# ReaganCardoza/Physics-Based-Ray-Tracing

Measured on AMD Instinct MI355X. Metric: Msamples/s on cbox.xml 512x512 x 256 spp (radiance, path max_depth 6), higher is better.
Workload: dtype f32

## Files before the change

### include/pbrt_hip.h

```cpp
#ifndef PBRT_HIP_H
#define PBRT_HIP_H

#include <stdint.h>

#ifdef __cplusplus
extern "C" {
#endif

#define PBRT_ABI_VERSION 5

#define PBRT_OK 0
#define PBRT_E_INVALID (-1)
#define PBRT_E_DEVICE (-2)
#define PBRT_E_NOMEM (-3)
#define PBRT_E_UNSUPPORTED (-4)

#define PBRT_PRIM_TRIANGLE 0u
#define PBRT_PRIM_SPHERE 1u
#define PBRT_PRIM_PARALLELOGRAM 2u
#define PBRT_PRIM_CONE 3u
#define PBRT_PRIM_CYLINDER 4u

typedef struct pbrt_prim {
    float g[12];
// ... 4 lines not shown
} pbrt_prim;

#define PBRT_MAT_DIFFUSE 0u
#define PBRT_MAT_CONDUCTOR 1u
#define PBRT_MAT_DIELECTRIC 2u
#define PBRT_MAT_ULTRA 3u
#define PBRT_MAT_NONE 4u
#define PBRT_MAT_ROUGHCONDUCTOR 5u
#define PBRT_MAT_CONDUCTOR_FRESNEL 6u

typedef struct pbrt_material {
    uint32_t type;
    float p[7];
} pbrt_material;

#define PBRT_EMIT_AREA 0u
#define PBRT_EMIT_POINT 1u

typedef struct pbrt_emitter {
    uint32_t type;
    float radiance[3];
    float pos[3];
    uint32_t first;
    uint32_t count;
    float area;
    float pad[2];
} pbrt_emitter;

#define PBRT_ACCEL_AUTO 0u
#define PBRT_ACCEL_BRUTE 1u
#define PBRT_ACCEL_BVH 2u
#define PBRT_ACCEL_BVH_GLOBAL 3u

typedef struct pbrt_scene_desc {
    uint32_t n_prims;
    const pbrt_prim *prims;
    uint32_t n_materials;
    const pbrt_material *materials;
    uint32_t n_emitters;
    const pbrt_emitter *emitters;
    uint32_t n_light_prims;
    const uint32_t *light_prims;
    const float *light_cdf;
    uint32_t accel;
    const float *vertex_normals;
} pbrt_scene_desc;

typedef struct pbrt_camera {
    float to_world[12];
    float tan_half_fov_x;
    float near_clip;
    float far_clip;
    uint32_t film_w;
    uint32_t film_h;
} pbrt_camera;

#define PBRT_FILTER_BOX 0u
#define PBRT_FILTER_TENT 1u
#define PBRT_FILTER_GAUSSIAN 2u

typedef struct pbrt_film_desc {
    uint32_t crop_x, crop_y, crop_w, crop_h;
    uint32_t spp;
    uint32_t sample_offset;
    uint32_t max_depth;
    uint32_t rr_depth;
    uint32_t filter;
    uint32_t seed;
    uint32_t flags;
    uint32_t pass_paths;
} pbrt_film_desc;

#define PBRT_FILM_RAW_ACCUM 1u
#define PBRT_FILM_NO_REPACK 2u
#define PBRT_FILM_FUSE_PLAN_SET 0x80u
#define PBRT_FILM_FUSE_PLAN(mask) (PBRT_FILM_FUSE_PLAN_SET | (((mask) & 0xffu) << 8))
#define PBRT_FILM_WALK_SET 0x10000u
#define PBRT_FILM_WALK_FROM(d) (PBRT_FILM_WALK_SET | (((d) & 0xffu) << 17))
#define PBRT_FILM_REGEN 8u
#define PBRT_FILM_NO_HIT_POOL 0x10u
#define PBRT_FILM_NO_OCCLUDER_PRUNING 4u
#define PBRT_FILM_NO_TILE_CULL 0x20u
#define PBRT_FILM_NO_ORDERED_WALK 0x40u

#define PBRT_US_MAX_ANGLES 64

typedef struct pbrt_us_emitter {
    uint32_t number_of_elements;
    float pitch, element_width, element_height;
    float radius;
    float opening_angle;
    uint32_t number_of_rays_per_element;
    float speed_of_sound;
    float steering_angle_min, steering_angle_max;
} pbrt_us_emitter;

#define PBRT_US_PRIMARY_ELEMENT 0u
#define PBRT_US_PRIMARY_EMITTER 1u
#define PBRT_US_ARRAY_CONVEX 0x100u

typedef struct pbrt_us_params {
    uint32_t max_depth;
    float frequency;
    float sound_speed;
    float attenuation;
    float main_beam_angle;
    float cutoff_angle;
    float fs;
    uint32_t n_elements;
    float pitch;
    uint32_t n_angles;
    float angles_deg[PBRT_US_MAX_ANGLES];
    uint32_t time_samples;
    float sensor_to_world[12];
    float max_path_len;
    uint32_t quirks;
    uint32_t primary;
    pbrt_us_emitter emitter;
} pbrt_us_params;

#define PBRT_USQ_DIAG_SAMPLE 0x1u
#define PBRT_USQ_REF_REFLECT 0x2u
#define PBRT_USQ_UNIT_GGX_PDF 0x4u
#define PBRT_USQ_DOUBLE_LOCAL 0x8u
#define PBRT_USQ_MIXED_FRAMES 0x10u
#define PBRT_USQ_NEVER_ENTER 0x20u
#define PBRT_USQ_CLAMP_TIME 0x40u
#define PBRT_USQ_NO_TOF_ACCUM 0x80u
#define PBRT_USQ_NO_CARRIER 0x100u
#define PBRT_USQ_NO_FIRST_TABLES 0x200u
#define PBRT_USQ_NO_FUSED_BOUNCES 0x400u
#define PBRT_USQ_FROZEN_DRAWS 0x800u
#define PBRT_USQ_SIGNED_RR 0x1000u
#define PBRT_USQ_DRJIT_VARIANT (PBRT_USQ_CLAMP_TIME | PBRT_USQ_NO_TOF_ACCUM | PBRT_USQ_FROZEN_DRAWS | PBRT_USQ_SIGNED_RR)
#define PBRT_USQ_REFERENCE                                                                \
    (PBRT_USQ_DIAG_SAMPLE | PBRT_USQ_REF_REFLECT | PBRT_USQ_UNIT_GGX_PDF | PBRT_USQ_DOUBLE_LOCAL | \
     PBRT_USQ_MIXED_FRAMES | PBRT_USQ_NEVER_ENTER)

typedef struct pbrt_us_sensor {
    uint32_t num_elements;
    float element_width, element_height, pitch;
    float radius;
    float center_frequency, sound_speed, directivity;
    float to_world[12];
} pbrt_us_sensor;

typedef struct pbrt_us_receiver {
    uint32_t number_of_elements;
    float pitch;
    float sample_rate;
    uint32_t time_samples;
} pbrt_us_receiver;

typedef struct pbrt_stats {
    uint64_t samples;
    uint64_t segments;
    uint64_t shadow_rays;
    double kernel_ms;
    double bounce_ms;
    uint32_t bounce_launches;
    uint32_t passes;
    uint64_t model_bytes;
    uint64_t bounce_model_bytes;
    uint64_t live[16];
    uint32_t fuse_plan;
    uint32_t plan_source;
// ... 223 lines not shown
```

### physics-based-ray-tracing_amd/_capi.py

```python
from __future__ import annotations

import contextlib
import ctypes as C
import os
import sys

import numpy as np

_HERE = os.path.dirname(os.path.abspath(__file__))
LIB_PATH = os.environ.get("PBRT_HIP_LIB") or os.path.join(_HERE, "csrc", "libpbrt_hip.so")

PBRT_ABI_VERSION = 5

PRIM_TRIANGLE, PRIM_SPHERE, PRIM_PARALLELOGRAM, PRIM_CONE, PRIM_CYLINDER = 0, 1, 2, 3, 4
MAT_DIFFUSE, MAT_CONDUCTOR, MAT_DIELECTRIC, MAT_ULTRA, MAT_NONE = 0, 1, 2, 3, 4
MAT_ROUGHCONDUCTOR, MAT_CONDUCTOR_FRESNEL = 5, 6
EMIT_AREA, EMIT_POINT = 0, 1
ACCEL_AUTO, ACCEL_BRUTE, ACCEL_BVH, ACCEL_BVH_GLOBAL = 0, 1, 2, 3
FILTER_BOX, FILTER_TENT, FILTER_GAUSSIAN = 0, 1, 2
FILM_RAW_ACCUM = 1
FILM_NO_REPACK = 2
FILM_NO_OCCLUDER_PRUNING = 4
FILM_NO_TILE_CULL = 0x20
FILM_NO_ORDERED_WALK = 0x40
FILM_NO_HIT_POOL = 0x10
FILM_REGEN = 8
FILM_FUSE_PLAN_SET = 0x80


FILM_WALK_SET = 0x10000


def film_walk_from(depth: int) -> int:
    return FILM_WALK_SET | ((int(depth) & 0xFF) << 17)


def film_fuse_plan(mask: int) -> int:
    return FILM_FUSE_PLAN_SET | ((int(mask) & 0xFF) << 8)

US_MAX_ANGLES = 64

USQ_DIAG_SAMPLE = 0x1
USQ_REF_REFLECT = 0x2
USQ_UNIT_GGX_PDF = 0x4
USQ_DOUBLE_LOCAL = 0x8
USQ_MIXED_FRAMES = 0x10
USQ_NEVER_ENTER = 0x20
USQ_CLAMP_TIME = 0x40
USQ_NO_TOF_ACCUM = 0x80
USQ_NO_CARRIER = 0x100
USQ_NO_FIRST_TABLES = 0x200
USQ_NO_FUSED_BOUNCES = 0x400
USQ_FROZEN_DRAWS = 0x800
USQ_SIGNED_RR = 0x1000
USQ_DRJIT_VARIANT = USQ_CLAMP_TIME | USQ_NO_TOF_ACCUM | USQ_FROZEN_DRAWS | USQ_SIGNED_RR
USQ_REFERENCE = (USQ_DIAG_SAMPLE | USQ_REF_REFLECT | USQ_UNIT_GGX_PDF | USQ_DOUBLE_LOCAL
                 | USQ_MIXED_FRAMES | USQ_NEVER_ENTER)

PRIM_DTYPE = np.dtype([("g", np.float32, 12), ("type", np.uint32), ("material", np.uint32),
                       ("emitter", np.int32), ("shape", np.uint32)])
MATERIAL_DTYPE = np.dtype([("type", np.uint32), ("p", np.float32, 7)])
EMITTER_DTYPE = np.dtype([("type", np.uint32), ("radiance", np.float32, 3), ("pos", np.float32, 3),
                          ("first", np.uint32), ("count", np.uint32), ("area", np.float32),
                          ("pad", np.float32, 2)])
assert PRIM_DTYPE.itemsize == 64 and MATERIAL_DTYPE.itemsize == 32 and EMITTER_DTYPE.itemsize == 48


class Material(C.Structure):
    _fields_ = [("type", C.c_uint32), ("p", C.c_float * 7)]


class SceneDesc(C.Structure):
    _fields_ = [("n_prims", C.c_uint32), ("prims", C.c_void_p),
                ("n_materials", C.c_uint32), ("materials", C.c_void_p),
                ("n_emitters", C.c_uint32), ("emitters", C.c_void_p),
                ("n_light_prims", C.c_uint32), ("light_prims", C.c_void_p), ("light_cdf", C.c_void_p),
                ("accel", C.c_uint32), ("vertex_normals", C.c_void_p)]


class Camera(C.Structure):
    _fields_ = [("to_world", C.c_float * 12), ("tan_half_fov_x", C.c_float), ("near_clip", C.c_float),
                ("far_clip", C.c_float), ("film_w", C.c_uint32), ("film_h", C.c_uint32)]


class FilmDesc(C.Structure):
    _fields_ = [("crop_x", C.c_uint32), ("crop_y", C.c_uint32), ("crop_w", C.c_uint32), ("crop_h", C.c_uint32),
                ("spp", C.c_uint32), ("sample_offset", C.c_uint32), ("max_depth", C.c_uint32),
                ("rr_depth", C.c_uint32), ("filter", C.c_uint32), ("seed", C.c_uint32), ("flags", C.c_uint32),
                ("pass_paths", C.c_uint32)]


class UsEmitter(C.Structure):
    _fields_ = [("number_of_elements", C.c_uint32), ("pitch", C.c_float), ("element_width", C.c_float),
                ("element_height", C.c_float), ("radius", C.c_float), ("opening_angle", C.c_float),
                ("number_of_rays_per_element", C.c_uint32), ("speed_of_sound", C.c_float),
                ("steering_angle_min", C.c_float), ("steering_angle_max", C.c_float)]


class UsParams(C.Structure):
    _fields_ = [("max_depth", C.c_uint32), ("frequency", C.c_float), ("sound_speed", C.c_float),
                ("attenuation", C.c_float), ("main_beam_angle", C.c_float), ("cutoff_angle", C.c_float),
                ("fs", C.c_float), ("n_elements", C.c_uint32), ("pitch", C.c_float), ("n_angles", C.c_uint32),
                ("angles_deg", C.c_float * US_MAX_ANGLES), ("time_samples", C.c_uint32),
                ("sensor_to_world", C.c_float * 12), ("max_path_len", C.c_float), ("quirks", C.c_uint32),
                ("primary", C.c_uint32), ("emitter", UsEmitter)]


# ... 460 lines not shown
```

### physics-based-ray-tracing_amd/csrc/diag_driver.h

```cpp
#pragma once

#ifndef PBRT_DEFAULT_WALK_FROM
#define PBRT_DEFAULT_WALK_FROM 0xffu
#endif

static RadKern diag_walk_kernel(const pbrt_scene *s, bool first, uint32_t nb) {
    return with_flags(
        [](auto F, auto B, auto N) -> RadKern { return &k_walk<F(), B() ? ACCEL_K_BRUTE_BIG : ACCEL_K_BRUTE, N() ? 2 : 1>; }, first,
        s->accel_kernel != ACCEL_K_BRUTE, nb == 2);
}
static RadKern diag_bvh_kernel(const pbrt_scene *s, bool first) {
    return with_flags([](auto F, auto L) -> RadKern { return &k_bounce<F(), L() ? ACCEL_K_BVH_LDS : ACCEL_K_BVH_GLOBAL>; }, first,
                      s->accel_kernel == ACCEL_K_BVH_LDS);
}
static UsKern diag_us_bvh_kernel(const pbrt_scene *s, bool first, bool convex) {
    return with_flags([](auto F, auto L, auto X) -> UsKern {
        return &k_us_bounce<F(), L() ? ACCEL_K_BVH_LDS : ACCEL_K_BVH_GLOBAL, false, US_Q_RUNTIME, -1, X()>; },
                      first, s->accel_kernel == ACCEL_K_BVH_LDS, convex);
}
static int diag_lds_attr(pbrt_scene *s, bool us) {
    if (s->accel_kernel != ACCEL_K_BVH_LDS) return PBRT_OK;
    for (bool first : {true, false}) {
        if (!us) {
            HIPCHK(s->ctx, set_max_lds(diag_bvh_kernel(s, first), s->lds_bytes));
// ... 61 lines not shown
            hipLaunchKernelGGL(k_regen<ACCEL_K_BRUTE_BIG>, dim3(grid), dim3(REGEN_WG), 0, st, a);
        HIPCHK(c, hipGetLastError());
        ++r.launches;
        return PBRT_OK;
    }
    for (uint32_t depth = 0; depth < f->max_depth;) {
        const uint32_t nb = brute ? chain_len(r.plan, depth, f->max_depth) : 1u;
        a.depth = depth;
        a.nb = nb;
        a.in = in;
        a.out = out;
        a.seg_in = sin;
        a.seg_out = sout;
        if (dg.repack && depth >= 2) {
            const uint32_t owners = rad_owners_per_region(s->accel_kernel), wreg = r.region / owners;
            const uint32_t n_own_pass = nseg_pass * owners;
            hipLaunchKernelGGL(k_scan_owners, dim3(1), dim3(1024), 0, st, sin, n_own_pass, wreg, owners, (uint32_t)c->n_cu, dg.offs,
                               dg.segC, dg.quota);
            hipLaunchKernelGGL(k_repack_copy, dim3(n_own_pass), dim3(256), 0, st, in, dg.stC, sin, dg.offs, dg.quota, n_own_pass, wreg);
            a.in = dg.stC;
            a.seg_in = dg.segC;
        }
        if (depth == 0 && (rc = r.timer.begin()) != 0) return rc;
        const bool walk = brute && depth >= dg.walk_from;
        const uint32_t pair_m = (brute && depth == 0 && !walk) ? pair_merge_bounce(dg.pair_merge, r.plan, f->max_depth) : 0u;
        if (pair_m) {
            a.merge_at = pair_m;
            const uint32_t g2 = div_up(a.n_paths, 2u * SEG_BRUTE);
            if (s->accel_kernel == ACCEL_K_BRUTE)
                hipLaunchKernelGGL(k_chain_pair<ACCEL_K_BRUTE>, dim3(g2), dim3(SEG_BRUTE), 0, st, a);
            else
                hipLaunchKernelGGL(k_chain_pair<ACCEL_K_BRUTE_BIG>, dim3(g2), dim3(SEG_BRUTE), 0, st, a);
        } else if (walk || !brute) {
            const RadKern k = walk ? diag_walk_kernel(s, depth == 0, nb) : diag_bvh_kernel(s, depth == 0);
            const bool lds = s->accel_kernel == ACCEL_K_BVH_LDS;
            hipLaunchKernelGGL(k, dim3(nseg_pass), dim3(seg_threads(s->accel_kernel)), lds ? s->lds_bytes : 0u, st, a);
        } else if ((rc = launch_bounce(s, a, nseg_pass, depth == 0, nb)) != 0) {
            return rc;
        }
        HIPCHK(c, hipGetLastError());
        ++r.launches;
        if (walk) break;
        std::swap(in, out);
        std::swap(sin, sout);
        const uint32_t depth_before = depth;
        depth += nb;
        bool dead;
        if ((rc = poll_live(c, f->max_depth, depth_before, depth, sin, r.n_own, &dead)) != 0) return rc;
        if (dead) break;
    }
    return PBRT_OK;
}

static int diag_render(Render &r) {
    pbrt_ctx *c = r.c;
    const pbrt_film_desc *f = r.f;
    int rc;
    if (!r.brute && (rc = diag_lds_attr(r.s, false)) != 0) return rc;
    if ((rc = render_buffers(r)) != 0) return rc;
    if (f->flags & (PBRT_FILM_WALK_SET | PBRT_FILM_REGEN)) r.probe = false;
    DiagRender dg;
    dg.pair_merge = diag_pair_merge();
    if (f->flags & PBRT_FILM_WALK_SET) dg.walk_from = (f->flags >> 17) & 0xffu;
    dg.repack = !r.brute && rad_wave_private(r.s->accel_kernel) && !(f->flags & PBRT_FILM_NO_REPACK);
    if (dg.repack) {
        dg.stC = (float *)c->buf("stateC", (size_t)r.cap * N_STATE * 4);
        dg.segC = (uint32_t *)c->buf("segC", (size_t)r.n_own * 4);
        dg.offs = (uint32_t *)c->buf("seg_offs", (size_t)r.n_own * 4);
        dg.quota = (uint32_t *)c->buf("seg_quota", 64);
        if (!dg.stC || !dg.segC || !dg.offs || !dg.quota) return PBRT_E_NOMEM;
    }
    if ((rc = render_args(r)) != 0) return rc;
    uint32_t s_step = r.s_pass;
    for (uint32_t s0 = 0; s0 < f->spp; ++r.passes) {
        const bool probing = r.probe && r.passes == 0;
        const uint32_t sc = probing ? PROBE_SPP : std::min(s_step, f->spp - s0);
        RadArgs a = r.base;
        a.n_paths = (uint32_t)(r.npix_r * sc);
        a.s_first = f->sample_offset + s0;
        if ((rc = diag_pass(r, dg, a, div_up(a.n_paths, r.region))) != 0) return rc;
        if ((rc = r.timer.end()) != 0) return rc;
        r.fa.s_first = a.s_first;
        r.fa.s_count = sc;
        film_accum(c, r.fa);
        HIPCHK(c, hipGetLastError());
        s0 += sc;
        if (probing) {
            if ((rc = probe_plan(c, r.segstats, r.n_rows, r.stat_rows, r.dstats, f->max_depth, &r.plan)) != 0) return rc;
            const uint32_t rem = f->spp - s0;
            s_step = div_up(rem, div_up(rem, r.s_pass));
        }
    }
    if ((rc = render_finish(r)) != 0) return rc;
    if (r.brute && (f->flags & PBRT_FILM_REGEN)) {
        pbrt_stats &S = c->stats;
        S.model_bytes = S.model_bytes - S.bounce_model_bytes + S.samples * 12;
        S.bounce_model_bytes = S.samples * 12;
    }
    return PBRT_OK;
}
```

### physics-based-ray-tracing_amd/csrc/kernels_radiance.h

```cpp
#pragma once
#include "device_scene.h"
#include "tile_cull.h"

#ifndef SEG_BRUTE
#define SEG_BRUTE 512
#endif
#ifndef SEG_BVH
#define SEG_BVH 1024
#endif
#ifndef SEG_WAVES_PER_EU
#define SEG_WAVES_PER_EU 8
#endif
#ifndef REGION_SEGS_BVH
#define REGION_SEGS_BVH 4
#endif
#ifndef REGION_SEGS_BRUTE
#define REGION_SEGS_BRUTE 1
#endif
#ifndef REGION_SEGS_US
#define REGION_SEGS_US 8
#endif
__host__ __device__ constexpr uint32_t rad_region_segs(int accel);
#ifndef REGION_SEGS_US_EMIT
#define REGION_SEGS_US_EMIT 16
// ... 597 lines not shown
    const unsigned long long *row = stats + (size_t)blockIdx.x * stride;
    const uint32_t per = (nseg + gridDim.y - 1) / gridDim.y, lo = min(blockIdx.y * per, nseg), hi = min(lo + per, nseg);
    unsigned long long s = 0;
    for (uint32_t i = lo + threadIdx.x; i < hi; i += 256) s += row[i];
    part[threadIdx.x] = s;
    __syncthreads();
    for (uint32_t w = 128; w > 0; w >>= 1) {
        if (threadIdx.x < w) part[threadIdx.x] += part[threadIdx.x + w];
        __syncthreads();
    }
    if (threadIdx.x == 0 && part[0]) atomicAdd(&out[blockIdx.x], part[0]);
}

__global__ __launch_bounds__(256) void k_us_reduce_stats(unsigned long long *stats, uint32_t nseg, size_t stride,
                                                         unsigned long long *out) {
    __shared__ unsigned long long part[4];
    unsigned long long *row = stats + (size_t)blockIdx.x * stride;
    const uint32_t per = (nseg + gridDim.y - 1) / gridDim.y, lo = min(blockIdx.y * per, nseg), hi = min(lo + per, nseg);
    unsigned long long s = 0;
    for (uint32_t i = lo + threadIdx.x; i < hi; i += 256) {
        s += row[i];
        row[i] = 0ull;
    }
#pragma unroll
    for (int off = 32; off > 0; off >>= 1) s += __shfl_xor(s, off);
    if ((threadIdx.x & 63u) == 0u) part[threadIdx.x >> 6] = s;
    __syncthreads();
    if (threadIdx.x == 0) out[(size_t)blockIdx.x * gridDim.y + blockIdx.y] = part[0] + part[1] + part[2] + part[3];
}

struct FilmArgs {
    const float *Lhome;
    float *acc;
    uint32_t cap;
    uint32_t cx0, cy0, cw, ch;
    uint32_t rx0, ry0, rw, rh;
    uint32_t npix_r, s_first, s_count, film_w, film_h, filter, seed;
    uint32_t tile_rows;
};

DEV float filter_1d(uint32_t f, float x) {
    if (f == PBRT_FILTER_TENT) return fmaxf(0.0f, 1.0f - fabsf(x));
    const float alpha = -2.0f;
    return fmaxf(0.0f, expf(alpha * x * x) - expf(alpha * 4.0f));
}

__global__ __launch_bounds__(256) void k_film_accum(const FilmArgs a) {
    const uint32_t idx = blockIdx.x * blockDim.x + threadIdx.x;
    if (idx >= a.cw * a.ch) return;
    const uint32_t iy = idx / a.cw, ix = idx - iy * a.cw;
    const int x = (int)(a.cx0 + ix), y = (int)(a.cy0 + iy);
    const uint32_t npx = a.cw * a.ch;
    float ar = a.acc[idx], ag = a.acc[npx + idx], ab = a.acc[2 * npx + idx], aw = a.acc[3 * npx + idx];
    const int R = a.filter == PBRT_FILTER_BOX ? 0 : (a.filter == PBRT_FILTER_TENT ? 1 : 2);
    const float ccx = (float)x + 0.5f, ccy = (float)y + 0.5f;
    for (uint32_t sl = 0; sl < a.s_count; ++sl) {
        const uint32_t s_idx = a.s_first + sl;
        const float4 *Ls = reinterpret_cast<const float4 *>(a.Lhome) + (size_t)sl * a.npix_r;
        for (int ny = y - R; ny <= y + R; ++ny)
            for (int nx = x - R; nx <= x + R; ++nx) {
                if (nx < 0 || ny < 0 || nx >= (int)a.film_w || ny >= (int)a.film_h) continue;
                float w = 1.0f;
                if (a.filter != PBRT_FILTER_BOX) {
                    F4 uj = rng4((uint32_t)ny * a.film_w + (uint32_t)nx, s_idx, 0, a.seed);
                    float px = (float)nx + uj.x, py = (float)ny + uj.y;
                    w = filter_1d(a.filter, ccx - px) * filter_1d(a.filter, ccy - py);
                }
                if (w > 0.0f) {
                    const uint32_t k = region_index((uint32_t)(nx - (int)a.rx0), (uint32_t)(ny - (int)a.ry0), a.rw, a.tile_rows);
                    const float4 Lk = Ls[k];
                    ar = fma_(w, Lk.x, ar);
                    ag = fma_(w, Lk.y, ag);
                    ab = fma_(w, Lk.z, ab);
                    aw += w;
                }
            }
    }
    a.acc[idx] = ar;
    a.acc[npx + idx] = ag;
    a.acc[2 * npx + idx] = ab;
    a.acc[3 * npx + idx] = aw;
}

#define FILM_RMAX 2
template <int FILM_TILE, int FILTER>
__global__ __launch_bounds__(FILM_TILE *FILM_TILE) void k_film_accum_tiled(const FilmArgs a) {
    constexpr int FILM_TW = FILM_TILE + 2 * FILM_RMAX;
    constexpr int LS = FILM_TILE == 16 ? 48 : 40;
    static_assert(LS >= FILM_TW, "row stride covers the haloed row");
    __shared__ float tile[2][5][FILM_TW * LS];
    constexpr int R = FILTER == PBRT_FILTER_TENT ? 1 : 2;
    constexpr int TW = FILM_TILE + 2 * R;
    const uint32_t tid = threadIdx.y * FILM_TILE + threadIdx.x;
    const int tx0 = (int)(a.cx0 + blockIdx.x * FILM_TILE), ty0 = (int)(a.cy0 + blockIdx.y * FILM_TILE);
    const int x = tx0 + (int)threadIdx.x, y = ty0 + (int)threadIdx.y;
    const bool inside = x < (int)(a.cx0 + a.cw) && y < (int)(a.cy0 + a.ch);
    const uint32_t npx = a.cw * a.ch;
    const uint32_t idx = inside ? (uint32_t)(y - (int)a.cy0) * a.cw + (uint32_t)(x - (int)a.cx0) : 0u;
    float ar = 0, ag = 0, ab = 0, aw = 0;
    if (inside) {
        ar = a.acc[idx];
        ag = a.acc[npx + idx];
        ab = a.acc[2 * npx + idx];
        aw = a.acc[3 * npx + idx];
    }
    const float ccx = (float)x + 0.5f, ccy = (float)y + 0.5f;
    constexpr int NT = FILM_TILE * FILM_TILE, NST = (FILM_TW * FILM_TW + NT - 1) / NT;
    bool st_in[NST], st_valid[NST];
    uint32_t st_key[NST], st_k[NST];
    float st_x[NST], st_y[NST];
    int st_lds[NST];
#pragma unroll
    for (int j = 0; j < NST; ++j) {
        const int i = (int)tid + j * NT;
        const int nx = tx0 - R + i % TW, ny = ty0 - R + i / TW;
        st_lds[j] = (i / TW) * LS + i % TW;
        st_in[j] = i < TW * TW;
        st_valid[j] = st_in[j] && nx >= (int)a.rx0 && ny >= (int)a.ry0 && nx < (int)(a.rx0 + a.rw) && ny < (int)(a.ry0 + a.rh);
        st_key[j] = (uint32_t)ny * a.film_w + (uint32_t)nx;
        st_k[j] = st_valid[j] ? region_index((uint32_t)(nx - (int)a.rx0), (uint32_t)(ny - (int)a.ry0), a.rw, a.tile_rows) : 0u;
        st_x[j] = (float)nx;
        st_y[j] = (float)ny;
    }
    const float4 *Lrec = reinterpret_cast<const float4 *>(a.Lhome);
    const float4 zero4 = {0.0f, 0.0f, 0.0f, 0.0f};
#ifndef FILM_PF
#define FILM_PF 4
#endif
    constexpr int PF = FILM_PF;
    float4 Lq[PF][NST];
#pragma unroll
    for (int u = 0; u < PF; ++u)
#pragma unroll
        for (int j = 0; j < NST; ++j)
            Lq[u][j] = (st_valid[j] && (uint32_t)u < a.s_count) ? Lrec[(size_t)u * a.npix_r + st_k[j]] : zero4;
    for (uint32_t sl0 = 0; sl0 < a.s_count; sl0 += PF) {
#pragma unroll
        for (int u = 0; u < PF; ++u) {
            const uint32_t sl = sl0 + (uint32_t)u;
            if (sl >= a.s_count) break;
            const uint32_t s_idx = a.s_first + sl;
            float(*T)[FILM_TW * LS] = tile[sl & 1];
#pragma unroll
            for (int j = 0; j < NST; ++j) {
                if (!st_in[j]) continue;
                const int i = st_lds[j];
                float px = 1e30f, py = 1e30f;
                if (st_valid[j]) {
                    F4 uj = rng4(st_key[j], s_idx, 0, a.seed);
                    px = st_x[j] + uj.x;
                    py = st_y[j] + uj.y;
                }
                T[0][i] = px;
                T[1][i] = py;
                T[2][i] = Lq[u][j].x;
                T[3][i] = Lq[u][j].y;
                T[4][i] = Lq[u][j].z;
            }
#pragma unroll
            for (int j = 0; j < NST; ++j)
                Lq[u][j] = (st_valid[j] && sl + PF < a.s_count) ? Lrec[(size_t)(sl + PF) * a.npix_r + st_k[j]] : zero4;
            __syncthreads();
            if (inside) {
                const int e0 = (int)threadIdx.y * LS + (int)threadIdx.x;
#pragma unroll
                for (int dy = 0; dy <= 2 * R; ++dy)
#pragma unroll
                    for (int dx = 0; dx <= 2 * R; ++dx) {
                        const int e = e0 + dy * LS + dx;
                        float w = filter_1d(FILTER, ccx - T[0][e]) * filter_1d(FILTER, ccy - T[1][e]);
                        if (w > 0.0f) {
                            ar = fma_(w, T[2][e], ar);
                            ag = fma_(w, T[3][e], ag);
                            ab = fma_(w, T[4][e], ab);
                            aw += w;
                        }
                    }
            }
        }
    }
    if (inside) {
        a.acc[idx] = ar;
        a.acc[npx + idx] = ag;
        a.acc[2 * npx + idx] = ab;
        a.acc[3 * npx + idx] = aw;
    }
}

__global__ __launch_bounds__(256) void k_film_resolve(const float *acc, float *out, uint32_t npx, uint32_t raw) {
    const uint32_t idx = blockIdx.x * blockDim.x + threadIdx.x;
    if (idx >= npx) return;
    float r = acc[idx], g = acc[npx + idx], b = acc[2 * npx + idx], w = acc[3 * npx + idx];
    if (raw) {
        out[4 * idx] = r;
        out[4 * idx + 1] = g;
        out[4 * idx + 2] = b;
        out[4 * idx + 3] = w;
    } else {
        float inv = w > 0.0f ? 1.0f / w : 0.0f;
        out[3 * idx] = r * inv;
        out[3 * idx + 1] = g * inv;
        out[3 * idx + 2] = b * inv;
    }
}

__global__ __launch_bounds__(256) void k_init_rays(float *st, uint32_t *seg_cnt, uint32_t n_cnt, uint32_t region, uint32_t n,
                                                   const float *o, const float *d, const float *tmax) {
    const uint32_t i = blockIdx.x * blockDim.x + threadIdx.x;
    if (i < n_cnt) seg_cnt[i] = n > i * region ? min(n - i * region, region) : 0u;
    if (i >= n) return;
    float *s = st + (state_voff(i) >> 2);
    s[0 * 64] = o[i];
    s[1 * 64] = o[n + i];
    s[2 * 64] = o[2 * n + i];
    s[3 * 64] = d[i];
    s[4 * 64] = d[n + i];
    s[5 * 64] = d[2 * n + i];
    s[6 * 64] = 1.0f;
    s[7 * 64] = 1.0f;
    s[8 * 64] = 1.0f;
    s[9 * 64] = 0.0f;
    s[10 * 64] = 0.0f;
    s[11 * 64] = 0.0f;
    s[12 * 64] = tmax[i];
    s[13 * 64] = -1.0f;
    s[14 * 64] = __uint_as_float(i);
}
```

### physics-based-ray-tracing_amd/csrc/pbrt_api.hip

```cpp
#include <hip/hip_runtime.h>

#include <atomic>
#include <cmath>
#include <cstdarg>
#include <cstdio>
#include <cstring>
#include <map>
#include <numeric>
#include <string>
#include <tuple>
#include <vector>

#include "bvh_build.h"
#include "prim_runs.h"
#include "bf_request.h"
#include "us_request.h"
#include "kernels_us.h"
#include "kernels_wavefront.h"
#include "kernels_us_wavefront.h"
#include "kernels_beamform.h"
#ifdef PBRT_DIAG
#include "kernels_diag.h"
#endif
#include "stage_layout.h"
// ... 1004 lines not shown
            float t = 0.0f;
            HIPCHK(c, hipEventElapsedTime(&t, c->ev_pool[i], c->ev_pool[i + 1]));
            bounce_ms += t;
        }
    }
    pbrt_stats &S = c->stats;
    S = pbrt_stats{};
    S.samples = samples;
    S.segments = hstats[0];
    S.shadow_rays = hstats[1];
    S.kernel_ms = ms;
    S.bounce_ms = bounce_ms;
    S.bounce_launches = launches;
    S.passes = passes;
    for (int d = 0; d < 16; ++d) S.live[d] = hstats[2 + d];
    S.workspace_bytes = c->work.total();
    return PBRT_OK;
}

static const uint64_t PASS_MIN_PATHS = 1u << 20;
#ifndef US_PASS_PATHS
#define US_PASS_PATHS (16u << 20)
#endif
struct PassShape {
    uint32_t per_pass = 1, cap = 0, nseg = 0;
};
template <typename Alloc>
static int size_pass(pbrt_ctx *c, uint64_t pass_paths, bool fixed, uint32_t per_call, uint64_t unit, uint32_t region, bool equal,
                     Alloc alloc, PassShape *ps) {
    for (;;) {
        uint32_t k = (uint32_t)std::max<uint64_t>(1, std::min<uint64_t>(per_call, pass_paths / std::max<uint64_t>(unit, 1)));
        if (equal) k = div_up(per_call, div_up(per_call, k));
        NEED(c, unit * k < 0xfffffc00ull);
        ps->per_pass = k;
        ps->cap = div_up(unit * k, region) * region;
        ps->nseg = ps->cap / region;
        const int rc = alloc(ps->cap, ps->nseg);
        if (rc != PBRT_E_NOMEM) return rc;
        release_pass_buffers(c);
        if (fixed || k <= 1 || pass_paths <= PASS_MIN_PATHS) return PBRT_E_NOMEM;
        pass_paths = std::max<uint64_t>(PASS_MIN_PATHS, std::min<uint64_t>(pass_paths, unit * k) / 2);
    }
}
static uint64_t default_pass_paths(pbrt_ctx *c, bool streams, uint64_t paths, uint32_t bytes_per_path) {
    if (streams) return wf_default_pass_paths(c, PASS_MIN_PATHS);
    if (c->work.limit)
        while (paths > PASS_MIN_PATHS && (double)paths * (double)bytes_per_path > (double)c->work.limit - 64e6) paths /= 2;
    return paths;
}

static bool fastdiv_exact(const FastDiv &fd, uint32_t d, std::initializer_list<uint32_t> probes) {
    for (uint32_t n : probes)
        if (udiv_fast_host(n, fd) != n / d) return false;
    return true;
}

static WfArgs wf_args(const RadArgs &a) {
    WfArgs w{};
    w.sc = a.sc;
    w.cam = a.cam;
    w.Lhome = a.Lhome;
    w.stats = a.stats;
    w.stat_stride = a.stat_stride;
    w.cap = a.cap;
    w.n_paths = a.n_paths;
    w.max_depth = a.max_depth;
    w.rr_depth = a.rr_depth;
    w.seed = a.seed;
    w.key_mode = a.key_mode;
    w.rx0 = a.rx0;
    w.ry0 = a.ry0;
    w.rw = a.rw;
    w.npix_r = a.npix_r;
    w.s_first = a.s_first;
    w.film_w = a.film_w;
    w.film_h = a.film_h;
    w.tile_rows = a.tile_rows;
    w.div_npix = a.div_npix;
    w.div_rw = a.div_rw;
    w.index_offset = a.index_offset;
    w.sample_index = a.sample_index;
    return w;
}
static void film_accum(pbrt_ctx *c, const FilmArgs &fa) {
    hipStream_t st = c->stream;
    if (fa.filter == PBRT_FILTER_BOX) {
        hipLaunchKernelGGL(k_film_accum, dim3(div_up((uint64_t)fa.cw * fa.ch, 256)), dim3(256), 0, st, fa);
        return;
    }
    const bool big = (uint64_t)div_up(fa.cw, 16) * div_up(fa.ch, 16) >= 4ull * (uint64_t)c->n_cu;
    const bool tent = fa.filter == PBRT_FILTER_TENT;
    const dim3 g16(div_up(fa.cw, 16), div_up(fa.ch, 16)), g8(div_up(fa.cw, 8), div_up(fa.ch, 8));
    if (big && tent)
        hipLaunchKernelGGL((k_film_accum_tiled<16, PBRT_FILTER_TENT>), g16, dim3(16, 16), 0, st, fa);
    else if (big)
        hipLaunchKernelGGL((k_film_accum_tiled<16, PBRT_FILTER_GAUSSIAN>), g16, dim3(16, 16), 0, st, fa);
    else if (tent)
        hipLaunchKernelGGL((k_film_accum_tiled<8, PBRT_FILTER_TENT>), g8, dim3(8, 8), 0, st, fa);
    else
        hipLaunchKernelGGL((k_film_accum_tiled<8, PBRT_FILTER_GAUSSIAN>), g8, dim3(8, 8), 0, st, fa);
}

static int probe_plan(pbrt_ctx *c, unsigned long long *segstats, uint32_t n_rows, uint32_t stat_rows, unsigned long long *dstats,
                      uint32_t max_depth, uint32_t *plan) {
    hipStream_t st = c->stream;
    unsigned long long hp[2 + MAX_DEPTH_STATS];
    hipLaunchKernelGGL(k_reduce_stats, dim3(stat_rows, REDUCE_SLICES), dim3(256), 0, st, segstats, n_rows, (size_t)n_rows, dstats);
    HIPCHK(c, hipGetLastError());
    HIPCHK(c, hipMemcpyAsync(hp, dstats, (size_t)stat_rows * 8, hipMemcpyDeviceToHost, st));
    HIPCHK(c, hipStreamSynchronize(st));
    HIPCHK(c, hipMemsetAsync(dstats, 0, (2 + 2 * MAX_DEPTH_STATS) * 8, st));
    for (uint32_t d = stat_rows; d < 2 + MAX_DEPTH_STATS; ++d) hp[d] = 0;
    *plan = plan_from_survival(hp + 2, std::min<uint32_t>(max_depth, MAX_DEPTH_STATS));
    return PBRT_OK;
}

namespace {
struct Render {
    pbrt_scene *s;
    pbrt_ctx *c;
    const pbrt_camera *cam;
    const pbrt_film_desc *f;
    void *d_out;
    bool brute = false, wavefront = false;
    Switches sw;
    uint32_t rx0 = 0, ry0 = 0, rw = 0, rh = 0;
    uint64_t npix_r = 0, film_px = 0;
    uint32_t region = 0, s_pass = 0, cap = 0, nseg = 0;
    uint32_t n_own = 0, n_rows = 0, stat_rows = 0, hit_rows = 0;
    WfBufs wfb{};
    WfPlan wfp;
    float *Lhome = nullptr, *acc = nullptr;
    uint32_t *segA = nullptr, *segB = nullptr;
    unsigned long long *dstats = nullptr, *segstats = nullptr;
    RadArgs base{};
    FilmArgs fa{};
    PassTimer timer{};
    uint32_t passes = 0, launches = 0, plan = 0;
    bool probe = false, plan_was_learnt = false;
};
}
constexpr uint32_t PROBE_SPP = 2;

static int render_check(Render &r) {
    pbrt_ctx *c = r.c;
    const pbrt_camera *cam = r.cam;
    const pbrt_film_desc *f = r.f;
    void *d_out = r.d_out;
    if (int rcs = ctx_settle(c)) return rcs;
    NEED(c, cam && f && d_out);
    const uint32_t W = cam->film_w, H = cam->film_h;
    NEED(c, W > 0 && H > 0 && f->crop_w > 0 && f->crop_h > 0);
    NEED(c, (uint64_t)f->crop_x + f->crop_w <= W && (uint64_t)f->crop_y + f->crop_h <= H);
    NEED(c, f->spp > 0 && f->max_depth > 0 && f->filter <= PBRT_FILTER_GAUSSIAN);
    NEED(c, (uint64_t)W * H <= 0xffffffffull);
    HIPCHK(c, hipSetDevice(c->device));
    r.brute = r.s->accel_kernel == ACCEL_K_BRUTE || r.s->accel_kernel == ACCEL_K_BRUTE_BIG;
    r.wavefront = !r.brute && !(f->flags & PBRT_FILM_NO_HIT_POOL);
    r.sw = read_switches();
    const uint32_t R = f->filter == PBRT_FILTER_BOX ? 0 : (f->filter == PBRT_FILTER_TENT ? 1 : 2);
    r.rx0 = f->crop_x > R ? f->crop_x - R : 0;
    r.ry0 = f->crop_y > R ? f->crop_y - R : 0;
    const uint32_t rx1 = std::min(f->crop_x + f->crop_w + R, W), ry1 = std::min(f->crop_y + f->crop_h + R, H);
    r.rw = rx1 - r.rx0;
    r.rh = ry1 - r.ry0;
    r.npix_r = (uint64_t)r.rw * r.rh;
    r.film_px = (uint64_t)f->crop_w * f->crop_h;
    return PBRT_OK;
}

static int render_buffers(Render &r) {
    pbrt_scene *s = r.s;
    pbrt_ctx *c = r.c;
    const pbrt_film_desc *f = r.f;
    const bool brute = r.brute, wavefront = r.wavefront;
    const uint64_t pass_paths = f->pass_paths ? f->pass_paths
                                              : default_pass_paths(c, wavefront, brute ? (64u << 20) : (16u << 20), 16 + 2 * N_STATE * 4);
    static_assert(WF_REGION == REGION_SEGS_BVH * SEG_BVH, "both BVH launch structures cut a pass into the same regions");
    r.region = rad_region_segs(s->accel_kernel) * seg_threads(s->accel_kernel);
    auto alloc_pass = [&](uint32_t cap, uint32_t nseg) -> int {
        NEED(c, wavefront || (uint64_t)cap * N_STATE * 4 < 0xffffffffull);
        if (wavefront) NEED(c, cap < WF_DEAD);
        r.Lhome = (float *)c->buf("Lhome", (size_t)cap * 16);
        return r.Lhome && (!wavefront || wf_alloc(c, cap, nseg, &r.wfb)) ? PBRT_OK : PBRT_E_NOMEM;
    };
    PassShape ps;
    int rc;
    if ((rc = size_pass(c, pass_paths, f->pass_paths != 0, f->spp, r.npix_r, r.region, true, alloc_pass, &ps)) != 0) return rc;
    r.s_pass = ps.per_pass;
    r.cap = ps.cap;
    r.nseg = ps.nseg;
    if (wavefront) {
        r.wfp = wf_plan(s, r.sw);
        if ((rc = wf_set_attr(s, r.wfp)) != 0) return rc;
    }
    r.n_own = r.nseg * rad_owners_per_region(s->accel_kernel);
    r.segA = (uint32_t *)c->buf("segA", (size_t)r.n_own * 4);
    r.segB = (uint32_t *)c->buf("segB", (size_t)r.n_own * 4);
    r.acc = (float *)c->buf("film_acc", r.film_px * 16);
    r.dstats = (unsigned long long *)c->buf("stats", (2 + 2 * MAX_DEPTH_STATS) * 8);
    r.n_rows = r.nseg * (wavefront ? WF_SHADE_THREADS / 64u : rad_rows_per_region(s->accel_kernel));
    r.stat_rows = 2 + (uint32_t)std::min<uint64_t>(f->max_depth, MAX_DEPTH_STATS);
    const size_t segstats_bytes = (size_t)r.stat_rows * r.n_rows * 8;
    r.segstats = (unsigned long long *)c->buf("segstats", (size_t)(2 + 2 * MAX_DEPTH_STATS) * r.n_rows * 8);
    if (!r.segstats) return PBRT_E_NOMEM;
    if (!r.Lhome || !r.segA || !r.segB || !r.acc || !r.dstats) return PBRT_E_NOMEM;
    r.hit_rows = wavefront ? r.stat_rows - 2 : 0;
    hipStream_t st = c->stream;
    HIPCHK(c, hipMemsetAsync(r.acc, 0, r.film_px * 16, st));
    HIPCHK(c, hipMemsetAsync(r.dstats, 0, (2 + 2 * MAX_DEPTH_STATS) * 8, st));
    HIPCHK(c, hipMemsetAsync(r.segstats, 0, segstats_bytes, st));
    if (r.hit_rows) HIPCHK(c, hipMemsetAsync(r.segstats + (size_t)HIT_ROW0 * r.n_rows, 0, (size_t)r.hit_rows * r.n_rows * 8, st));
    HIPCHK(c, hipEventRecord(c->ev0, st));
    r.timer = PassTimer{c};
    r.plan_was_learnt = brute && s->plan_hint_valid;
    r.plan = !brute ? 0u
             : (f->flags & PBRT_FILM_FUSE_PLAN_SET) ? ((f->flags >> 8) & 0xffu)
             : (s->plan_hint_valid ? s->plan_hint : PBRT_DEFAULT_FUSE_PLAN);
    r.probe = brute && !s->plan_hint_valid && f->spp >= 8 * PROBE_SPP && r.s_pass >= PROBE_SPP && !(f->flags & PBRT_FILM_FUSE_PLAN_SET);
    return PBRT_OK;
}

static int render_args(Render &r) {
    pbrt_scene *s = r.s;
    pbrt_ctx *c = r.c;
    const pbrt_film_desc *f = r.f;
    const uint32_t rw = r.rw, cap = r.cap;
    RadArgs &base = r.base;
    base.sc = s->ds;
    if ((f->flags & PBRT_FILM_NO_OCCLUDER_PRUNING) && base.sc.occ_prims) {
        base.sc.occ_prims = base.sc.prims;
        base.sc.n_occ = base.sc.n_prims;
        base.sc.occ_runs = base.sc.prim_runs;
        base.sc.n_occ_runs = base.sc.n_prim_runs;
        base.sc.occ_ord = base.sc.prim_ord;
    }
    if (f->flags & PBRT_FILM_NO_ORDERED_WALK) base.sc.prim_ord = base.sc.occ_ord = 0u;
    base.cam = *r.cam;
// ... 50 lines not shown
            key.rh = r.rh;
        }
        base.tile_keep = ta.keep;
        c->tile_keep_last = true;
        c->tile_keep_words = ta.keep;
    }
    FilmArgs &fa = r.fa;
    fa.Lhome = r.Lhome;
    fa.acc = r.acc;
    fa.cap = cap;
    fa.cx0 = f->crop_x;
    fa.cy0 = f->crop_y;
    fa.cw = f->crop_w;
    fa.ch = f->crop_h;
    fa.rx0 = r.rx0;
    fa.ry0 = r.ry0;
    fa.rw = rw;
    fa.rh = r.rh;
    fa.npix_r = (uint32_t)r.npix_r;
    fa.tile_rows = base.tile_rows;
    fa.film_w = r.cam->film_w;
    fa.film_h = r.cam->film_h;
    fa.filter = f->filter;
    fa.seed = f->seed;
    return PBRT_OK;
}

constexpr uint32_t PASS_MAX_BOUNCES = 256;
static int brute_pass(Render &r, RadArgs a, uint32_t nseg_pass) {
    pbrt_ctx *c = r.c;
    const uint32_t max_depth = r.f->max_depth;
    const bool one_launch = chain_len(r.plan, 0, max_depth) >= max_depth;
    const size_t need = one_launch ? (size_t)r.region : (size_t)nseg_pass * r.region;
    float *in = (float *)c->buf("stateA", need * N_STATE * 4), *out = (float *)c->buf("stateB", need * N_STATE * 4);
    if (!in || !out) return PBRT_E_NOMEM;
    a.state_cap = (uint32_t)need;
    uint32_t *sin = r.segA, *sout = r.segB;
    int rc;
    if ((rc = r.timer.begin()) != 0) return rc;
    for (uint32_t depth = 0; depth < max_depth && depth < PASS_MAX_BOUNCES;) {
        const uint32_t nb = chain_len(r.plan, depth, max_depth);
        a.depth = depth;
        a.nb = nb;
        a.in = in;
        a.out = out;
        a.seg_in = sin;
        a.seg_out = sout;
        if ((rc = launch_bounce(r.s, a, nseg_pass, depth == 0, nb)) != 0) return rc;
        HIPCHK(c, hipGetLastError());
        ++r.launches;
        std::swap(in, out);
        std::swap(sin, sout);
        const uint32_t depth_before = depth;
        depth += nb;
        bool dead;
        if ((rc = poll_live(c, max_depth, depth_before, depth, sin, r.n_own, &dead)) != 0) return rc;
        if (dead) break;
    }
    return PBRT_OK;
}

static int render_passes(Render &r) {
    pbrt_ctx *c = r.c;
    const pbrt_film_desc *f = r.f;
    int rc;
    uint32_t s_step = r.s_pass;
    for (uint32_t s0 = 0; s0 < f->spp; ++r.passes) {
        const bool probing = r.probe && r.passes == 0;
        const uint32_t sc = probing ? PROBE_SPP : std::min(s_step, f->spp - s0);
        RadArgs a = r.base;
        a.n_paths = (uint32_t)(r.npix_r * sc);
        a.s_first = f->sample_offset + s0;
        const uint32_t nseg_pass = div_up(a.n_paths, r.region);
        if (r.wavefront) {
            if ((rc = r.timer.begin()) != 0) return rc;
            rc = wf_bounces(r.s, wf_args(a), r.wfb, r.wfp, nseg_pass, true, &r.launches);
        } else {
            rc = brute_pass(r, a, nseg_pass);
        }
        if (rc) return rc;
        if ((rc = r.timer.end()) != 0) return rc;
        r.fa.s_first = a.s_first;
        r.fa.s_count = sc;
        film_accum(c, r.fa);
        HIPCHK(c, hipGetLastError());
        s0 += sc;
        if (probing) {
            if ((rc = probe_plan(c, r.segstats, r.n_rows, r.stat_rows, r.dstats, f->max_depth, &r.plan)) != 0) return rc;
            const uint32_t rem = f->spp - s0;
            s_step = div_up(rem, div_up(rem, r.s_pass));
        }
    }
    return PBRT_OK;
}

static int render_finish(Render &r) {
    pbrt_scene *s = r.s;
    pbrt_ctx *c = r.c;
    const pbrt_film_desc *f = r.f;
    const bool wavefront = r.wavefront;
    const uint32_t n_rows = r.n_rows;
    hipStream_t st = c->stream;
    int rc;
    hipLaunchKernelGGL(k_film_resolve, dim3(div_up(r.film_px, 256)), dim3(256), 0, st, r.acc, (float *)r.d_out, (uint32_t)r.film_px,
                       (uint32_t)((f->flags & PBRT_FILM_RAW_ACCUM) ? 1 : 0));
    HIPCHK(c, hipGetLastError());
    HIPCHK(c, hipEventRecord(c->ev1, st));
    unsigned long long hstats[2 + 2 * MAX_DEPTH_STATS];
    hipLaunchKernelGGL(k_reduce_stats, dim3(r.stat_rows, REDUCE_SLICES), dim3(256), 0, st, r.segstats, n_rows, (size_t)n_rows, r.dstats);
    if (r.hit_rows)
        hipLaunchKernelGGL(k_reduce_stats, dim3(r.hit_rows, REDUCE_SLICES), dim3(256), 0, st, r.segstats + (size_t)HIT_ROW0 * n_rows, n_rows,
                           (size_t)n_rows, r.dstats + HIT_ROW0);
    HIPCHK(c, hipGetLastError());
    HIPCHK(c, hipMemcpyAsync(hstats, r.dstats, sizeof hstats, hipMemcpyDeviceToHost, st));
    uint32_t hguard[WF_GUARD_WORDS] = {0};
    if (wavefront && (rc = wf_guard_fetch(c, hguard)) != 0) return rc;
    HIPCHK(c, hipStreamSynchronize(st));
    if (wavefront && (rc = wf_check_guard(c, hguard)) != 0) return rc;
    if ((rc = call_stats(c, hstats, r.npix_r * f->spp, r.launches, r.passes, true, r.timer.n_ev)) != 0) return rc;
    pbrt_stats &S = c->stats;
    S.fuse_plan = r.plan;
    S.plan_source = wavefront ? PBRT_PLAN_STREAMS
                    : (f->flags & PBRT_FILM_FUSE_PLAN_SET) ? PBRT_PLAN_CALLER
                    : r.probe ? PBRT_PLAN_PROBED
                    : r.plan_was_learnt ? PBRT_PLAN_LEARNT : PBRT_PLAN_DEFAULT;
    S.pass_paths = (uint64_t)r.npix_r * r.s_pass;
    if (r.brute && hstats[2] > 0) {
        s->plan_hint = plan_from_survival(hstats + 2, (uint32_t)std::min<uint64_t>(f->max_depth, MAX_DEPTH_STATS));
        s->plan_hint_valid = true;
    }
    uint64_t tot, bb;
    radiance_model_bytes(hstats + 2, MAX_DEPTH_STATS, S.samples, r.film_px, r.passes, r.plan, f->max_depth,
                         wavefront ? hstats + HIT_ROW0 : nullptr, &tot, &bb);
    if (wavefront) {
        tot -= bb;
        uint64_t trb = 0;
        bb = wavefront_model_bytes(hstats + 2, hstats + HIT_ROW0, MAX_DEPTH_STATS, S.shadow_rays, &trb);
        tot += bb;
        S.trace_model_bytes = trb;
    }
    S.model_bytes = tot;
    S.bounce_model_bytes = bb;
    return PBRT_OK;
}

#ifdef PBRT_DIAG
#include "diag_driver.h"
#endif

static int render_impl(pbrt_scene *s, const pbrt_camera *cam, const pbrt_film_desc *f, void *d_out) {
    Render r{s, s->ctx, cam, f, d_out};
    int rc;
    if ((rc = render_check(r)) != 0) return rc;
#ifdef PBRT_DIAG
    if (diag_selected(r)) return diag_render(r);
#else
    if ((f->flags & (PBRT_FILM_REGEN | PBRT_FILM_WALK_SET)) || (!r.brute && (f->flags & PBRT_FILM_NO_HIT_POOL)))
        return r.c->fail(PBRT_E_UNSUPPORTED, "PBRT_FILM_REGEN / PBRT_FILM_WALK_FROM / PBRT_FILM_NO_HIT_POOL select diagnostic launch "
                                             "structures: build libpbrt_hip_diag.so (make -C csrc diag)");
#endif
    if ((rc = render_buffers(r)) != 0) return rc;
    if ((rc = render_args(r)) != 0) return rc;
    if ((rc = render_passes(r)) != 0) return rc;
    return render_finish(r);
}

#ifdef PBRT_BVH_PROBE
// ... 1250 lines not shown
```

Measured before the change: 11350.

## Pack film-tile LDS into float4 planes and pipeline row reads in filter gather

```diff
diff --git a/include/pbrt_hip.h b/include/pbrt_hip.h
--- a/include/pbrt_hip.h
+++ b/include/pbrt_hip.h
@@ -110,6 +110,8 @@
 #define PBRT_FILM_NO_OCCLUDER_PRUNING 4u
 #define PBRT_FILM_NO_TILE_CULL 0x20u
 #define PBRT_FILM_NO_ORDERED_WALK 0x40u
+#define PBRT_FILM_TILE16 0x2000000u
+#define PBRT_FILM_TILE8 0x4000000u
 
 #define PBRT_US_MAX_ANGLES 64
 
diff --git a/physics-based-ray-tracing_amd/_capi.py b/physics-based-ray-tracing_amd/_capi.py
--- a/physics-based-ray-tracing_amd/_capi.py
+++ b/physics-based-ray-tracing_amd/_capi.py
@@ -23,6 +23,8 @@
 FILM_NO_OCCLUDER_PRUNING = 4
 FILM_NO_TILE_CULL = 0x20
 FILM_NO_ORDERED_WALK = 0x40
+FILM_TILE16 = 0x2000000
+FILM_TILE8 = 0x4000000
 FILM_NO_HIT_POOL = 0x10
 FILM_REGEN = 8
 FILM_FUSE_PLAN_SET = 0x80
diff --git a/physics-based-ray-tracing_amd/csrc/diag_driver.h b/physics-based-ray-tracing_amd/csrc/diag_driver.h
--- a/physics-based-ray-tracing_amd/csrc/diag_driver.h
+++ b/physics-based-ray-tracing_amd/csrc/diag_driver.h
@@ -167,7 +167,7 @@
         if ((rc = r.timer.end()) != 0) return rc;
         r.fa.s_first = a.s_first;
         r.fa.s_count = sc;
-        film_accum(c, r.fa);
+        film_accum(c, r.fa, r.f->flags);
         HIPCHK(c, hipGetLastError());
         s0 += sc;
         if (probing) {
diff --git a/physics-based-ray-tracing_amd/csrc/kernels_radiance.h b/physics-based-ray-tracing_amd/csrc/kernels_radiance.h
--- a/physics-based-ray-tracing_amd/csrc/kernels_radiance.h
+++ b/physics-based-ray-tracing_amd/csrc/kernels_radiance.h
@@ -703,15 +703,16 @@
     a.acc[3 * npx + idx] = aw;
 }
 
-#define FILM_RMAX 2
+typedef float film_f4 __attribute__((ext_vector_type(4)));
 template <int FILM_TILE, int FILTER>
-__global__ __launch_bounds__(FILM_TILE *FILM_TILE) void k_film_accum_tiled(const FilmArgs a) {
-    constexpr int FILM_TW = FILM_TILE + 2 * FILM_RMAX;
-    constexpr int LS = FILM_TILE == 16 ? 48 : 40;
-    static_assert(LS >= FILM_TW, "row stride covers the haloed row");
-    __shared__ float tile[2][5][FILM_TW * LS];
+__global__ __launch_bounds__(FILM_TILE *FILM_TILE, (FILM_TILE == 8 && FILTER == PBRT_FILTER_GAUSSIAN) ? 3 : 4)
+void k_film_accum_tiled(const FilmArgs a) {
     constexpr int R = FILTER == PBRT_FILTER_TENT ? 1 : 2;
     constexpr int TW = FILM_TILE + 2 * R;
+    constexpr int LS4 = FILM_TILE == 16 ? 32 : 24, LS1 = FILM_TILE == 16 ? 48 : 40;
+    static_assert(LS4 >= TW && LS1 >= TW, "row strides cover the haloed row");
+    __shared__ film_f4 tile_pg[2][TW * LS4];
+    __shared__ float tile_b[2][TW * LS1];
     const uint32_t tid = threadIdx.y * FILM_TILE + threadIdx.x;
     const int tx0 = (int)(a.cx0 + blockIdx.x * FILM_TILE), ty0 = (int)(a.cy0 + blockIdx.y * FILM_TILE);
     const int x = tx0 + (int)threadIdx.x, y = ty0 + (int)threadIdx.y;
@@ -726,16 +727,17 @@
         aw = a.acc[3 * npx + idx];
     }
     const float ccx = (float)x + 0.5f, ccy = (float)y + 0.5f;
-    constexpr int NT = FILM_TILE * FILM_TILE, NST = (FILM_TW * FILM_TW + NT - 1) / NT;
+    constexpr int NT = FILM_TILE * FILM_TILE, NST = (TW * TW + NT - 1) / NT;
     bool st_in[NST], st_valid[NST];
     uint32_t st_key[NST], st_k[NST];
     float st_x[NST], st_y[NST];
-    int st_lds[NST];
+    int st_e4[NST], st_e1[NST];
 #pragma unroll
     for (int j = 0; j < NST; ++j) {
         const int i = (int)tid + j * NT;
         const int nx = tx0 - R + i % TW, ny = ty0 - R + i / TW;
-        st_lds[j] = (i / TW) * LS + i % TW;
+        st_e4[j] = (i / TW) * LS4 + i % TW;
+        st_e1[j] = (i / TW) * LS1 + i % TW;
         st_in[j] = i < TW * TW;
         st_valid[j] = st_in[j] && nx >= (int)a.rx0 && ny >= (int)a.ry0 && nx < (int)(a.rx0 + a.rw) && ny < (int)(a.ry0 + a.rh);
         st_key[j] = (uint32_t)ny * a.film_w + (uint32_t)nx;
@@ -743,60 +745,78 @@
         st_x[j] = (float)nx;
         st_y[j] = (float)ny;
     }
-    const float4 *Lrec = reinterpret_cast<const float4 *>(a.Lhome);
-    const float4 zero4 = {0.0f, 0.0f, 0.0f, 0.0f};
+    const film_f4 *Lrec = reinterpret_cast<const film_f4 *>(a.Lhome);
+    const film_f4 zero4 = {0.0f, 0.0f, 0.0f, 0.0f};
 #ifndef FILM_PF
 #define FILM_PF 4
 #endif
     constexpr int PF = FILM_PF;
-    float4 Lq[PF][NST];
+    film_f4 Lq[PF][NST];
 #pragma unroll
     for (int u = 0; u < PF; ++u)
 #pragma unroll
-        for (int j = 0; j < NST; ++j)
-            Lq[u][j] = (st_valid[j] && (uint32_t)u < a.s_count) ? Lrec[(size_t)u * a.npix_r + st_k[j]] : zero4;
+        for (int j = 0; j < NST; ++j) {
+            Lq[u][j] = zero4;
+            if ((uint32_t)u < a.s_count) Lq[u][j] = Lrec[(size_t)u * a.npix_r + st_k[j]];
+        }
+    constexpr int ND = 2 * R + 1;
+    const int g4 = (int)threadIdx.y * LS4 + (int)threadIdx.x, g1 = (int)threadIdx.y * LS1 + (int)threadIdx.x;
     for (uint32_t sl0 = 0; sl0 < a.s_count; sl0 += PF) {
 #pragma unroll
         for (int u = 0; u < PF; ++u) {
             const uint32_t sl = sl0 + (uint32_t)u;
             if (sl >= a.s_count) break;
             const uint32_t s_idx = a.s_first + sl;
-            float(*T)[FILM_TW * LS] = tile[sl & 1];
+            film_f4 *TQ = tile_pg[sl & 1];
+            float *TB = tile_b[sl & 1];
 #pragma unroll
             for (int j = 0; j < NST; ++j) {
                 if (!st_in[j]) continue;
-                const int i = st_lds[j];
                 float px = 1e30f, py = 1e30f;
+                film_f4 L = zero4;
                 if (st_valid[j]) {
                     F4 uj = rng4(st_key[j], s_idx, 0, a.seed);
                     px = st_x[j] + uj.x;
                     py = st_y[j] + uj.y;
+                    L = Lq[u][j];
                 }
-                T[0][i] = px;
-                T[1][i] = py;
-                T[2][i] = Lq[u][j].x;
-                T[3][i] = Lq[u][j].y;
-                T[4][i] = Lq[u][j].z;
-            }
-#pragma unroll
-            for (int j = 0; j < NST; ++j)
-                Lq[u][j] = (st_valid[j] && sl + PF < a.s_count) ? Lrec[(size_t)(sl + PF) * a.npix_r + st_k[j]] : zero4;
+                TQ[st_e4[j]] = film_f4{px, py, L.x, L.y};
+                TB[st_e1[j]] = L.z;
+            }
+            if (sl + PF < a.s_count) {
+#pragma unroll
+                for (int j = 0; j < NST; ++j) Lq[u][j] = Lrec[(size_t)(sl + PF) * a.npix_r + st_k[j]];
+            }
             __syncthreads();
             if (inside) {
-                const int e0 = (int)threadIdx.y * LS + (int)threadIdx.x;
-#pragma unroll
-                for (int dy = 0; dy <= 2 * R; ++dy)
-#pragma unroll
-                    for (int dx = 0; dx <= 2 * R; ++dx) {
-                        const int e = e0 + dy * LS + dx;
-                        float w = filter_1d(FILTER, ccx - T[0][e]) * filter_1d(FILTER, ccy - T[1][e]);
+                constexpr int AH = FILTER == PBRT_FILTER_TENT ? 1 : 0;
+                const film_f4 *GQ = TQ + g4;
+                const float *GB = TB + g1;
+                film_f4 tq[2][ND];
+                float tb[2][ND];
+                auto read_row = [&](int r) {
+#pragma unroll
+                    for (int dx = 0; dx < ND; ++dx) {
+                        tq[r & 1][dx] = GQ[r * LS4 + dx];
+                        tb[r & 1][dx] = GB[r * LS1 + dx];
+                    }
+                };
+                if (AH) read_row(0);
+#pragma unroll
+                for (int dy = 0; dy < ND; ++dy) {
+                    if (dy + AH < ND) read_row(dy + AH);
+#pragma unroll
+                    for (int dx = 0; dx < ND; ++dx) {
+                        const film_f4 q = tq[dy & 1][dx];
+                        const float w = filter_1d(FILTER, ccx - q.x) * filter_1d(FILTER, ccy - q.y);
                         if (w > 0.0f) {
-                            ar = fma_(w, T[2][e], ar);
-                            ag = fma_(w, T[3][e], ag);
-                            ab = fma_(w, T[4][e], ab);
+                            ar = fma_(w, q.z, ar);
+                            ag = fma_(w, q.w, ag);
+                            ab = fma_(w, tb[dy & 1][dx], ab);
                             aw += w;
                         }
                     }
+                }
             }
         }
     }
diff --git a/physics-based-ray-tracing_amd/csrc/pbrt_api.hip b/physics-based-ray-tracing_amd/csrc/pbrt_api.hip
--- a/physics-based-ray-tracing_amd/csrc/pbrt_api.hip
+++ b/physics-based-ray-tracing_amd/csrc/pbrt_api.hip
@@ -1110,13 +1110,14 @@
     w.sample_index = a.sample_index;
     return w;
 }
-static void film_accum(pbrt_ctx *c, const FilmArgs &fa) {
+static void film_accum(pbrt_ctx *c, const FilmArgs &fa, uint32_t flags) {
     hipStream_t st = c->stream;
     if (fa.filter == PBRT_FILTER_BOX) {
         hipLaunchKernelGGL(k_film_accum, dim3(div_up((uint64_t)fa.cw * fa.ch, 256)), dim3(256), 0, st, fa);
         return;
     }
-    const bool big = (uint64_t)div_up(fa.cw, 16) * div_up(fa.ch, 16) >= 4ull * (uint64_t)c->n_cu;
+    const bool big = (flags & PBRT_FILM_TILE16) ||
+                     (!(flags & PBRT_FILM_TILE8) && (uint64_t)div_up(fa.cw, 16) * div_up(fa.ch, 16) >= 4ull * (uint64_t)c->n_cu);
     const bool tent = fa.filter == PBRT_FILTER_TENT;
     const dim3 g16(div_up(fa.cw, 16), div_up(fa.ch, 16)), g8(div_up(fa.cw, 8), div_up(fa.ch, 8));
     if (big && tent)
@@ -1182,6 +1183,8 @@
     NEED(c, (uint64_t)f->crop_x + f->crop_w <= W && (uint64_t)f->crop_y + f->crop_h <= H);
     NEED(c, f->spp > 0 && f->max_depth > 0 && f->filter <= PBRT_FILTER_GAUSSIAN);
     NEED(c, (uint64_t)W * H <= 0xffffffffull);
+    if ((f->flags & PBRT_FILM_TILE16) && (f->flags & PBRT_FILM_TILE8))
+        return c->fail(PBRT_E_INVALID, "PBRT_FILM_TILE16 and PBRT_FILM_TILE8 together: the film gather runs one tile size");
     HIPCHK(c, hipSetDevice(c->device));
     r.brute = r.s->accel_kernel == ACCEL_K_BRUTE || r.s->accel_kernel == ACCEL_K_BRUTE_BIG;
     r.wavefront = !r.brute && !(f->flags & PBRT_FILM_NO_HIT_POOL);
@@ -1398,7 +1401,7 @@
         if ((rc = r.timer.end()) != 0) return rc;
         r.fa.s_first = a.s_first;
         r.fa.s_count = sc;
-        film_accum(c, r.fa);
+        film_accum(c, r.fa, r.f->flags);
         HIPCHK(c, hipGetLastError());
         s0 += sc;
         if (probing) {
```

After: 11460, median of 6. No clear change (+0.9%).
